# ArjunNarayanan/ProximalPolicyOptimization.jl

Hardware: AMD Instinct MI355X
Metric: env-steps/sec end-to-end PPO (rollout+GAE+update), 4096 envs, 1/2/4/8 MI355X (higher is better)
Workload: dtype f32; 1 GPU; 4096 parallel synthetic rand-poly-shaped envs per GPU (Q=8,H=32,A=128,F=72 int8), 2x256 MLP policy fp32, T=128 steps/iteration, 4 epochs, minibatch 4096/GPU, gamma=1.0 eps=0.05 entropy_w=0.01 Adam 1e-4; returns mode (lambda=1,V=0); envs_per_gpu=4096, T=128, epochs=4, minibatch_per_gpu=4096, parallelism=dp1, rollouts_streamed_to_disk=False

## Files before the change

### proximalpolicyoptimization.jl_amd/csrc/ppo_policy_fwd_x6.hip

```cpp
#include "ppo_policy_tail.h"
#include "ppo_x6.h"
#include <cstdlib>

#define X6F_LANE() unsigned ln = (unsigned)lane; asm volatile("" : "+v"(ln)); const int j = (int)(ln & 31u), h = (int)(ln >> 5); (void)j; (void)h

template <int HID>
struct FXCfg {
    static constexpr int F = 72, NT = HID / 32, KS = HID / 16, K1 = 5;
    static constexpr size_t oFr = 0, szFr = (size_t)NT * 6 * 1024;
    static constexpr size_t oP = oFr + szFr, oW3 = oP + (size_t)NT * 1024, oB1 = oW3 + (size_t)2 * NT * 256,
                            oB2 = oB1 + (size_t)NT * 128, total = oB2 + (size_t)NT * 128;
    static constexpr int WG_PER_CU = HID == 256 ? 2 : 4;
    static_assert(total * WG_PER_CU <= 160 * 1024, "LDS budget");
};

template <int HID>
__global__ __launch_bounds__(HID * 2, 4) void k_policy_fwd_train_x6(FwdArgs a, const uint4* __restrict__ w1x, const uint4* __restrict__ w2fx, int x_by_tile) {
    using C = FXCfg<HID>;
    constexpr int F = C::F, NT = C::NT, KS = C::KS, K1 = C::K1;
    extern __shared__ __attribute__((aligned(16))) char smem_c[];
    char* const frag = smem_c + C::oFr;
    float4* const sP = reinterpret_cast<float4*>(smem_c + C::oP);
    float4* const sW3p = reinterpret_cast<float4*>(smem_c + C::oW3);
    float4* const sB1 = reinterpret_cast<float4*>(smem_c + C::oB1);
    float4* const sB2 = reinterpret_cast<float4*>(smem_c + C::oB2);
    const int tid = threadIdx.x, lane = tid & 63;
    const int w = __builtin_amdgcn_readfirstlane(tid >> 6);
#ifdef PPO_X6_ZERO_LDS
    for (int i = tid; i < (int)(C::total / 4); i += NT * 64) reinterpret_cast<uint32_t*>(smem_c)[i] = 0u;
    __syncthreads();
#endif
    for (int i = tid; i < 2 * NT * 16; i += NT * 64) sW3p[i] = a.w3p[i];
    for (int i = tid; i < NT * 8; i += NT * 64) { sB1[i] = a.b1p[i]; sB2[i] = a.b2p[i]; }
    __syncthreads();
    const char* const w1s = reinterpret_cast<const char*>(w1x + (size_t)w * K1 * 3 * 64);
    const char* const w2s = reinterpret_cast<const char*>(w2fx + (size_t)w * KS * 3 * 64);
    char* const fown = frag + (size_t)w * 6 * 1024;

    uint2 xr[K1];
    auto load_x = [&](int64_t rec, unsigned ln) {
        const char* row = reinterpret_cast<const char*>(a.states) + (size_t)rec * 32 * F + (ln & 31u) * (unsigned)F + (ln >> 5) * 8u;
#pragma unroll
        for (int s = 0; s < K1; ++s) {
            const bool pad = (s == K1 - 1) && (ln >> 5);
            const uint2 v = *reinterpret_cast<const uint2*>(row + (pad ? 0 : 16 * s));
            xr[s] = pad ? make_uint2(0u, 0u) : v;
        }
    };
    int32_t sid = 0;
    if ((int64_t)blockIdx.x < a.B) { sid = __builtin_amdgcn_readfirstlane(a.idx[blockIdx.x]); load_x(x_by_tile ? (int64_t)blockIdx.x : (int64_t)sid, (unsigned)lane); }

    for (int64_t tile = blockIdx.x; tile < a.B; tile += gridDim.x) {
        const uint32_t act = a.active[sid];
        const int32_t sid_cur = sid;
        {
            X6F_LANE();
            unsigned lo16 = ln * 16u;
            constexpr int R1 = 8;
            uint4 ring[R1];
#pragma unroll
            for (int g = 0; g < R1; ++g) ring[g] = *reinterpret_cast<const uint4*>(w1s + (lo16 + (unsigned)g * 1024u));
            f32x16 acc;
#pragma unroll
            for (int q = 0; q < 4; ++q) {
                const float4 b = sB1[(w * 2 + h) * 4 + q];
                acc[4 * q + 0] = b.x; acc[4 * q + 1] = b.y; acc[4 * q + 2] = b.z; acc[4 * q + 3] = b.w;
            }
            uint4 xb[K1];
#pragma unroll
            for (int s = 0; s < K1; ++s) {
                float v[8];
#pragma unroll
                for (int e = 0; e < 8; ++e) v[e] = (float)(int)(int8_t)((e < 4 ? xr[s].x : xr[s].y) >> (8 * (e & 3)));
                xb[s] = make_uint4(x_perm(v[0], v[1]), x_perm(v[2], v[3]), x_perm(v[4], v[5]), x_perm(v[6], v[7]));
            }
            f32x16 accs;
#pragma unroll
            for (int r = 0; r < 16; ++r) accs[r] = 0.0f;
#pragma unroll
            for (int st = 0; st < 3 * K1; ++st) {
                if (st % 3 == 2) acc = x_mfma(ring[st % R1], xb[st / 3], acc);
                else accs = x_mfma(ring[st % R1], xb[st / 3], accs);
                __builtin_amdgcn_sched_barrier(0);
                if (st + R1 < 3 * K1) ring[st % R1] = *reinterpret_cast<const uint4*>(w1s + (lo16 + (unsigned)(st + R1) * 1024u));
                __builtin_amdgcn_sched_barrier(0);
            }
#pragma unroll
            for (int r = 0; r < 16; ++r) acc[r] = acc[r] + accs[r];
            asm volatile("" : "+v"(acc));
            lrelu16(acc);
            float4* dst = a.act1 + ((size_t)tile * NT + w) * 4 * 64;
#pragma unroll
            for (int q = 0; q < 4; ++q) {
                typedef float f32x4l __attribute__((ext_vector_type(4)));
                const f32x4l t = {acc[4 * q], acc[4 * q + 1], acc[4 * q + 2], acc[4 * q + 3]};
                __builtin_nontemporal_store(t, reinterpret_cast<f32x4l*>(dst + q * 64 + ln));
            }
#pragma unroll
            for (int s = 0; s < 2; ++s) {
                uint2 zh[2], zm[2], zl[2];
#pragma unroll
                for (int qq = 0; qq < 2; ++qq) {
                    const int q = 2 * s + qq;
                    const float hv[4] = {acc[4 * q], acc[4 * q + 1], acc[4 * q + 2], acc[4 * q + 3]};
                    x_split4(hv, zh[qq], zm[qq], zl[qq]);
                }
                *reinterpret_cast<uint4*>(fown + (s * 3 + 0) * 1024 + ln * 16) = make_uint4(zh[0].x, zh[0].y, zh[1].x, zh[1].y);
                *reinterpret_cast<uint4*>(fown + (s * 3 + 1) * 1024 + ln * 16) = make_uint4(zm[0].x, zm[0].y, zm[1].x, zm[1].y);
                *reinterpret_cast<uint4*>(fown + (s * 3 + 2) * 1024 + ln * 16) = make_uint4(zl[0].x, zl[0].y, zl[1].x, zl[1].y);
            }
        }
        constexpr int RD = 6;
        static_assert(RD % 3 == 0 && KS % (RD / 3) == 0, "ring rounds");
        static_assert(RD * 1024 <= PPO_X6_W2_PAD_BYTES, "the last ring round reads RD pieces past the end of the W2 stream");
        uint4 ring[RD];
        {
            unsigned lo = (unsigned)lane * 16u;
            asm volatile("" : "+v"(lo));
#pragma unroll
            for (int g = 0; g < RD; ++g) ring[g] = *reinterpret_cast<const uint4*>(w2s + (lo + (unsigned)g * 1024u));
        }
        const int64_t ntile = (tile + gridDim.x < a.B) ? tile + gridDim.x : tile;
        {
            unsigned ln2 = (unsigned)lane;
            asm volatile("" : "+v"(ln2));
            sid = __builtin_amdgcn_readfirstlane(a.idx[ntile]);
            load_x(x_by_tile ? ntile : (int64_t)sid, ln2);
        }
        __syncthreads();
        {
            X6F_LANE();
            f32x16 acc;
#pragma unroll
            for (int q = 0; q < 4; ++q) {
                const float4 b = sB2[(w * 2 + h) * 4 + q];
                acc[4 * q + 0] = b.x; acc[4 * q + 1] = b.y; acc[4 * q + 2] = b.z; acc[4 * q + 3] = b.w;
            }
            f32x16 accm, accl;
#pragma unroll
            for (int r = 0; r < 16; ++r) { accm[r] = 0.0f; accl[r] = 0.0f; }
            const unsigned lo16 = ln * 16u;
            const char* zp = frag + lo16;
            const char* wn = w2s + (size_t)RD * 1024;
#pragma unroll 1
            for (int k0 = 0; k0 < KS; k0 += RD / 3) {
#pragma unroll
                for (int u = 0; u < RD / 3; ++u) {
                    const uint4 z_h = *reinterpret_cast<const uint4*>(zp + (u * 3 + 0) * 1024);
                    const uint4 z_m = *reinterpret_cast<const uint4*>(zp + (u * 3 + 1) * 1024);
                    const uint4 z_l = *reinterpret_cast<const uint4*>(zp + (u * 3 + 2) * 1024);
                    accl = x_mfma(ring[3 * u + 0], z_h, accl);
                    __builtin_amdgcn_sched_barrier(0);
                    ring[3 * u + 0] = *reinterpret_cast<const uint4*>(wn + lo16);
                    __builtin_amdgcn_sched_barrier(0);
                    accl = x_mfma(ring[3 * u + 1], z_m, accl);
                    accm = x_mfma(ring[3 * u + 1], z_h, accm);
                    __builtin_amdgcn_sched_barrier(0);
                    ring[3 * u + 1] = *reinterpret_cast<const uint4*>(wn + 1024 + lo16);
                    __builtin_amdgcn_sched_barrier(0);
                    accl = x_mfma(ring[3 * u + 2], z_l, accl);
                    accm = x_mfma(ring[3 * u + 2], z_m, accm);
                    acc = x_mfma(ring[3 * u + 2], z_h, acc);
                    __builtin_amdgcn_sched_barrier(0);
                    ring[3 * u + 2] = *reinterpret_cast<const uint4*>(wn + 2048 + lo16);
                    wn += 3 * 1024;
                    __builtin_amdgcn_sched_barrier(0);
                }
                zp += (RD / 3) * 3 * 1024;
            }
#pragma unroll
            for (int r = 0; r < 16; ++r) acc[r] = acc[r] + (accm[r] + accl[r]);
            asm volatile("" : "+v"(acc));
            lrelu16(acc);
            float4* dst = a.act2 + ((size_t)tile * NT + w) * 4 * 64;
#pragma unroll
            for (int q = 0; q < 4; ++q) {
                typedef float f32x4l __attribute__((ext_vector_type(4)));
                const f32x4l t = {acc[4 * q], acc[4 * q + 1], acc[4 * q + 2], acc[4 * q + 3]};
                __builtin_nontemporal_store(t, reinterpret_cast<f32x4l*>(dst + q * 64 + ln));
            }
            float p0 = 0.f, p1 = 0.f, p2 = 0.f, p3 = 0.f;
            const float4* w3 = sW3p + (h * NT + w) * 16;
#pragma unroll
            for (int r = 0; r < 16; ++r) {
                const float4 wv = w3[r];
                p0 = fmaf(wv.x, acc[r], p0); p1 = fmaf(wv.y, acc[r], p1);
                p2 = fmaf(wv.z, acc[r], p2); p3 = fmaf(wv.w, acc[r], p3);
            }
            sP[w * 64 + ln] = make_float4(p0, p1, p2, p3);
        }
        __syncthreads();
        if (w == 0) {
            X6F_LANE();
            float4 s = sP[ln];
#pragma unroll
            for (int u = 1; u < NT; ++u) { const float4 q4 = sP[u * 64 + ln]; s.x += q4.x; s.y += q4.y; s.z += q4.z; s.w += q4.w; }
            float l[1][4];
            l[0][0] = (s.x + __shfl_xor(s.x, 32)) + a.b3[0];
            l[0][1] = (s.y + __shfl_xor(s.y, 32)) + a.b3[1];
            l[0][2] = (s.z + __shfl_xor(s.z, 32)) + a.b3[2];
            l[0][3] = (s.w + __shfl_xor(s.w, 32)) + a.b3[3];
            policy_tail<2, 1, false>(a, tile, sid_cur, act, l, (int)ln, j, h);
        }
    }
}

template <int HID, int T>
struct FXTCfg {
    static constexpr int F = 72, NT = HID / 32, KS = HID / 16, K1 = 5;
    static constexpr size_t oFr = 0, szFr = (size_t)T * NT * 6 * 1024;
    static constexpr size_t oP = oFr + szFr, oW3 = oP + (size_t)T * NT * 1024, oB1 = oW3 + (size_t)2 * NT * 256,
                            oB2 = oB1 + (size_t)NT * 128, total = oB2 + (size_t)NT * 128;
    static_assert(total <= 160 * 1024, "LDS budget");
};

template <int HID, int T>
__global__ __launch_bounds__(HID * 2, 2) void k_policy_fwd_train_x6t(FwdArgs a, const uint4* __restrict__ w1x, const uint4* __restrict__ w2fx, int x_by_tile) {
    using C = FXTCfg<HID, T>;
    constexpr int F = C::F, NT = C::NT, KS = C::KS, K1 = C::K1;
    static_assert(T <= NT, "one tail wave per tile");
    static_assert(T == 2, "two scalar id loads per pass; waves 0 and 1 run the tails");
    extern __shared__ __attribute__((aligned(16))) char smem_c[];
    char* const frag = smem_c + C::oFr;
    float4* const sP = reinterpret_cast<float4*>(smem_c + C::oP);
    float4* const sW3p = reinterpret_cast<float4*>(smem_c + C::oW3);
    float4* const sB1 = reinterpret_cast<float4*>(smem_c + C::oB1);
    float4* const sB2 = reinterpret_cast<float4*>(smem_c + C::oB2);
    const int tid = threadIdx.x, lane = tid & 63;
    const int w = __builtin_amdgcn_readfirstlane(tid >> 6);
#ifdef PPO_FX6_STAMP
    unsigned long long st_sum[8] = {0, 0, 0, 0, 0, 0, 0, 0}, st_t = clock64();
#define FXSTAMP(i) do { unsigned long long _n = clock64(); st_sum[i] += _n - st_t; st_t = _n; } while (0)
#else
#define FXSTAMP(i) do { } while (0)
#endif
    const float b3_0 = a.b3[0], b3_1 = a.b3[1], b3_2 = a.b3[2], b3_3 = a.b3[3];
    for (int i = tid; i < 2 * NT * 16; i += NT * 64) sW3p[i] = a.w3p[i];
    for (int i = tid; i < NT * 8; i += NT * 64) { sB1[i] = a.b1p[i]; sB2[i] = a.b2p[i]; }
    __syncthreads();
    const char* const w1s = reinterpret_cast<const char*>(w1x + (size_t)w * K1 * 3 * 64);
    const char* const w2s = reinterpret_cast<const char*>(w2fx + (size_t)w * KS * 3 * 64);

    uint2 xr[T][K1];
    auto load_x = [&](int i, int64_t rec, unsigned ln) {
        const uint64_t rb = x_uniform_addr(reinterpret_cast<const char*>(a.states) + (size_t)rec * 32 * F);
        const unsigned row = (ln & 31u) * (unsigned)F + (ln >> 5) * 8u;
#pragma unroll
        for (int s = 0; s < K1; ++s) {
            const bool pad = (s == K1 - 1) && (ln >> 5);
            unsigned ro = row + (pad ? 0u : 16u * s);
            asm volatile("" : "+v"(ro));
            typedef unsigned u32x2l __attribute__((ext_vector_type(2)));
            const u32x2l vv = *x_gptr<const u32x2l>(rb, ro);
            const uint2 v = make_uint2(vv.x, vv.y);
            xr[i][s] = pad ? make_uint2(0u, 0u) : v;
        }
    };
    auto tile_of = [&](int64_t g, int i) { const int64_t t = g * T + i; return t < a.B ? t : a.B - 1; };
    int cid[T] = {0, 0}, nid[T] = {0, 0};
    auto sload_ids = [&](int64_t g, int (&id)[T]) {
        const int32_t* const ip0 = a.idx + tile_of(g, 0);
        const int32_t* const ip1 = a.idx + tile_of(g, 1);
        asm volatile("s_load_dword %0, %2, 0x0\n\ts_load_dword %1, %3, 0x0\n\ts_waitcnt lgkmcnt(0)"
                     : "=&s"(id[0]), "=&s"(id[1]) : "s"(ip0), "s"(ip1) : "memory");
    };
    uint32_t tact = 0u, nact = 0u;
    TailPre tpre = {0, 0.0f, 0.0f}, npre = {0, 0.0f, 0.0f};
    auto load_tail_in = [&](const int (&id)[T], uint32_t& act, TailPre& pre) {
        const int32_t s = w == 1 ? id[1] : id[0];
        act = a.active[s]; pre.ab = a.actions[s]; pre.po = a.p_old[s]; pre.adv = a.adv[s];
    };
    if ((int64_t)blockIdx.x * T < a.B) {
        sload_ids(blockIdx.x, cid);
#pragma unroll
        for (int i = 0; i < T; ++i) load_x(i, x_by_tile ? tile_of(blockIdx.x, i) : (int64_t)cid[i], (unsigned)lane);
        load_tail_in(cid, tact, tpre);
    }
    for (int64_t g = blockIdx.x; g * T < a.B; g += gridDim.x) {
        {
            X6F_LANE();
            unsigned lo16 = ln * 16u;
            constexpr int R1 = 8;
            uint4 ring[R1];
#pragma unroll
            for (int q = 0; q < R1; ++q) ring[q] = *reinterpret_cast<const uint4*>(w1s + (lo16 + (unsigned)q * 1024u));
            f32x16 acc[T], accs[T];
            uint4 xb[T][K1];
#pragma unroll
            for (int i = 0; i < T; ++i) {
#pragma unroll
                for (int q = 0; q < 4; ++q) {
                    const float4 b = sB1[(w * 2 + h) * 4 + q];
                    acc[i][4 * q + 0] = b.x; acc[i][4 * q + 1] = b.y; acc[i][4 * q + 2] = b.z; acc[i][4 * q + 3] = b.w;
                }
#pragma unroll
                for (int r = 0; r < 16; ++r) accs[i][r] = 0.0f;
#pragma unroll
                for (int s = 0; s < K1; ++s) {
                    float v[8];
#pragma unroll
                    for (int e = 0; e < 8; ++e) v[e] = (float)(int)(int8_t)((e < 4 ? xr[i][s].x : xr[i][s].y) >> (8 * (e & 3)));
                    xb[i][s] = make_uint4(x_perm(v[0], v[1]), x_perm(v[2], v[3]), x_perm(v[4], v[5]), x_perm(v[6], v[7]));
                }
            }
#pragma unroll
            for (int st = 0; st < 3 * K1; ++st) {
#pragma unroll
                for (int i = 0; i < T; ++i) {
                    if (st % 3 == 2) acc[i] = x_mfma(ring[st % R1], xb[i][st / 3], acc[i]);
                    else accs[i] = x_mfma(ring[st % R1], xb[i][st / 3], accs[i]);
                }
                __builtin_amdgcn_sched_barrier(0);
                if (st + R1 < 3 * K1) ring[st % R1] = *reinterpret_cast<const uint4*>(w1s + (lo16 + (unsigned)(st + R1) * 1024u));
                __builtin_amdgcn_sched_barrier(0);
            }
            FXSTAMP(0);
#pragma unroll
            for (int i = 0; i < T; ++i) {
#pragma unroll
                for (int r = 0; r < 16; ++r) acc[i][r] = acc[i][r] + accs[i][r];
                asm volatile("" : "+v"(acc[i]));
                lrelu16(acc[i]);
                const int64_t tile = g * T + i;
                if (tile < a.B) {
                    const uint64_t dst = x_uniform_addr(a.act1 + ((size_t)tile * NT + w) * 4 * 64);
#pragma unroll
                    for (int q = 0; q < 4; ++q) {
                        typedef float f32x4l __attribute__((ext_vector_type(4)));
                        const f32x4l t = {acc[i][4 * q], acc[i][4 * q + 1], acc[i][4 * q + 2], acc[i][4 * q + 3]};
                        unsigned so = ln * 16u + (unsigned)q * 1024u;
                        asm volatile("" : "+v"(so));
                        __builtin_nontemporal_store(t, x_gptr<f32x4l>(dst, so));
                    }
                }
                char* const fown = frag + ((size_t)i * NT + w) * 6 * 1024;
#pragma unroll
                for (int s = 0; s < 2; ++s) {
                    uint2 zh[2], zm[2], zl[2];
#pragma unroll
                    for (int qq = 0; qq < 2; ++qq) {
                        const int q = 2 * s + qq;
                        const float hv[4] = {acc[i][4 * q], acc[i][4 * q + 1], acc[i][4 * q + 2], acc[i][4 * q + 3]};
                        x_split4(hv, zh[qq], zm[qq], zl[qq]);
                    }
                    *reinterpret_cast<uint4*>(fown + (s * 3 + 0) * 1024 + ln * 16) = make_uint4(zh[0].x, zh[0].y, zh[1].x, zh[1].y);
                    *reinterpret_cast<uint4*>(fown + (s * 3 + 1) * 1024 + ln * 16) = make_uint4(zm[0].x, zm[0].y, zm[1].x, zm[1].y);
                    *reinterpret_cast<uint4*>(fown + (s * 3 + 2) * 1024 + ln * 16) = make_uint4(zl[0].x, zl[0].y, zl[1].x, zl[1].y);
                }
            }
        }
        FXSTAMP(1);
        constexpr int RD = 6;
        static_assert(KS % (RD / 3) == 0, "ring rounds");
        static_assert(RD * 1024 <= PPO_X6_W2_PAD_BYTES, "the last ring round reads RD pieces past the end of the W2 stream");
        uint4 ring[RD];
        {
            unsigned lo = (unsigned)lane * 16u;
            asm volatile("" : "+v"(lo));
#pragma unroll
            for (int q = 0; q < RD; ++q) ring[q] = *reinterpret_cast<const uint4*>(w2s + (lo + (unsigned)q * 1024u));
        }
        {
            const int64_t gn = ((g + gridDim.x) * T < a.B) ? g + gridDim.x : g;
            unsigned ln2 = (unsigned)lane;
            asm volatile("" : "+v"(ln2));
            sload_ids(gn, nid);
#pragma unroll
            for (int i = 0; i < T; ++i) load_x(i, x_by_tile ? tile_of(gn, i) : (int64_t)nid[i], ln2);
            load_tail_in(nid, nact, npre);
        }
        FXSTAMP(2);
        __syncthreads();
        FXSTAMP(3);
        {
            X6F_LANE();
            f32x16 acc[T], accs[T];
#pragma unroll
            for (int i = 0; i < T; ++i) {
#pragma unroll
                for (int q = 0; q < 4; ++q) {
                    const float4 b = sB2[(w * 2 + h) * 4 + q];
                    acc[i][4 * q + 0] = b.x; acc[i][4 * q + 1] = b.y; acc[i][4 * q + 2] = b.z; acc[i][4 * q + 3] = b.w;
                }
#pragma unroll
                for (int r = 0; r < 16; ++r) accs[i][r] = 0.0f;
            }
            const unsigned lo16 = ln * 16u;
            const char* zp = frag + lo16;
            unsigned wo = (unsigned)RD * 1024u;
            asm volatile("" : "+s"(wo));
#pragma unroll 1
            for (int k0 = 0; k0 < KS; k0 += RD / 3) {
#pragma unroll
                for (int u = 0; u < RD / 3; ++u) {
                    const uint4 wl = ring[3 * u + 0], wm = ring[3 * u + 1], wh = ring[3 * u + 2];
#pragma unroll
                    for (int i = 0; i < T; ++i) {
                        const char* zi = zp + (size_t)i * NT * 6 * 1024;
                        const uint4 z_h = *reinterpret_cast<const uint4*>(zi + (u * 3 + 0) * 1024);
                        const uint4 z_m = *reinterpret_cast<const uint4*>(zi + (u * 3 + 1) * 1024);
                        const uint4 z_l = *reinterpret_cast<const uint4*>(zi + (u * 3 + 2) * 1024);
                        accs[i] = x_mfma(wl, z_h, accs[i]);
                        accs[i] = x_mfma(wm, z_m, accs[i]);
                        accs[i] = x_mfma(wm, z_h, accs[i]);
                        accs[i] = x_mfma(wh, z_l, accs[i]);
                        accs[i] = x_mfma(wh, z_m, accs[i]);
                        acc[i] = x_mfma(wh, z_h, acc[i]);
                    }
                    __builtin_amdgcn_sched_barrier(0);
                    ring[3 * u + 0] = *reinterpret_cast<const uint4*>(w2s + (lo16 + wo));
                    ring[3 * u + 1] = *reinterpret_cast<const uint4*>(w2s + (lo16 + wo + 1024u));
                    ring[3 * u + 2] = *reinterpret_cast<const uint4*>(w2s + (lo16 + wo + 2048u));
                    wo += 3 * 1024;
                    asm volatile("" : "+s"(wo));
                    __builtin_amdgcn_sched_barrier(0);
                }
                zp += (RD / 3) * 3 * 1024;
            }
            FXSTAMP(4);
#pragma unroll
            for (int i = 0; i < T; ++i) {
#pragma unroll
                for (int r = 0; r < 16; ++r) acc[i][r] = acc[i][r] + accs[i][r];
                asm volatile("" : "+v"(acc[i]));
                lrelu16(acc[i]);
                const int64_t tile = g * T + i;
                if (tile < a.B) {
                    const uint64_t dst = x_uniform_addr(a.act2 + ((size_t)tile * NT + w) * 4 * 64);
#pragma unroll
                    for (int q = 0; q < 4; ++q) {
                        typedef float f32x4l __attribute__((ext_vector_type(4)));
                        const f32x4l t = {acc[i][4 * q], acc[i][4 * q + 1], acc[i][4 * q + 2], acc[i][4 * q + 3]};
                        unsigned so = ln * 16u + (unsigned)q * 1024u;
                        asm volatile("" : "+v"(so));
                        __builtin_nontemporal_store(t, x_gptr<f32x4l>(dst, so));
                    }
                }
                float p0 = 0.f, p1 = 0.f, p2 = 0.f, p3 = 0.f;
                const float4* w3 = sW3p + (h * NT + w) * 16;
#pragma unroll
                for (int r = 0; r < 16; ++r) {
                    const float4 wv = w3[r];
                    p0 = fmaf(wv.x, acc[i][r], p0); p1 = fmaf(wv.y, acc[i][r], p1);
                    p2 = fmaf(wv.z, acc[i][r], p2); p3 = fmaf(wv.w, acc[i][r], p3);
                }
                sP[(i * NT + w) * 64 + ln] = make_float4(p0, p1, p2, p3);
            }
        }
        FXSTAMP(5);
        __syncthreads();
        FXSTAMP(6);
        if (w < T && g * T + w < a.B) {
            X6F_LANE();
            const int64_t tile = g * T + w;
            const int32_t sidw = w == 0 ? cid[0] : cid[1];
            const float4* sPi = sP + (size_t)w * NT * 64;
            float4 s = sPi[ln];
#pragma unroll
            for (int u = 1; u < NT; ++u) { const float4 q4 = sPi[u * 64 + ln]; s.x += q4.x; s.y += q4.y; s.z += q4.z; s.w += q4.w; }
            float l[1][4];
            l[0][0] = (s.x + __shfl_xor(s.x, 32)) + b3_0;
            l[0][1] = (s.y + __shfl_xor(s.y, 32)) + b3_1;
            l[0][2] = (s.z + __shfl_xor(s.z, 32)) + b3_2;
            l[0][3] = (s.w + __shfl_xor(s.w, 32)) + b3_3;
            policy_tail<2, 1, false>(a, tile, sidw, tact, l, (int)ln, j, h, 0u, 0, &tpre);
        }
        FXSTAMP(7);
        cid[0] = nid[0]; cid[1] = nid[1];
        tact = nact; tpre = npre;
    }
#ifdef PPO_FX6_STAMP
    if (a.stamps && lane == 0 && (w == 0 || w == NT - 1))
        for (int i = 0; i < 8; ++i) a.stamps[((size_t)blockIdx.x * 2 + (w ? 1 : 0)) * 8 + i] = st_sum[i];
#endif
#undef FXSTAMP
}

template <int HID, int TPS>
struct FXSCfg {
    static constexpr int F = 72, NT = HID / 32, KS = HID / 16, K1 = 5;
    static constexpr size_t oFr = 0, szFr = (size_t)2 * NT * 6 * 1024;
    static constexpr size_t oP = oFr + szFr, oW3 = oP + (size_t)TPS * NT * 1024, oB1 = oW3 + (size_t)2 * NT * 256,
                            oB2 = oB1 + (size_t)NT * 128, total = oB2 + (size_t)NT * 128;
    static_assert(total <= 160 * 1024, "LDS budget");
};

template <int HID, int TPS>
__global__ __launch_bounds__(HID * 2, 2) void k_policy_fwd_train_x6s(FwdArgs a, const uint4* __restrict__ w1x, const uint4* __restrict__ w2fx, int x_by_tile) {
    constexpr int T = 2;
    static_assert(TPS % T == 0, "tiles of a state in pairs");
    using C = FXSCfg<HID, TPS>;
    constexpr int F = C::F, NT = C::NT, KS = C::KS, K1 = C::K1;
    extern __shared__ __attribute__((aligned(16))) char smem_c[];
    char* const frag = smem_c + C::oFr;
    float4* const sP = reinterpret_cast<float4*>(smem_c + C::oP);
    float4* const sW3p = reinterpret_cast<float4*>(smem_c + C::oW3);
    float4* const sB1 = reinterpret_cast<float4*>(smem_c + C::oB1);
    float4* const sB2 = reinterpret_cast<float4*>(smem_c + C::oB2);
    const int tid = threadIdx.x, lane = tid & 63;
    const int w = __builtin_amdgcn_readfirstlane(tid >> 6);
    for (int i = tid; i < 2 * NT * 16; i += NT * 64) sW3p[i] = a.w3p[i];
    for (int i = tid; i < NT * 8; i += NT * 64) { sB1[i] = a.b1p[i]; sB2[i] = a.b2p[i]; }
    __syncthreads();
    const char* const w1s = reinterpret_cast<const char*>(w1x + (size_t)w * K1 * 3 * 64);
    const char* const w2s = reinterpret_cast<const char*>(w2fx + (size_t)w * KS * 3 * 64);

    uint2 xr[T][K1];
    auto load_x = [&](int i, int64_t rec, unsigned ln) {
        const char* row = reinterpret_cast<const char*>(a.states) + (size_t)rec * 32 * F + (ln & 31u) * (unsigned)F + (ln >> 5) * 8u;
#pragma unroll
        for (int s = 0; s < K1; ++s) {
            const bool pad = (s == K1 - 1) && (ln >> 5);
            const uint2 v = *reinterpret_cast<const uint2*>(row + (pad ? 0 : 16 * s));
            xr[i][s] = pad ? make_uint2(0u, 0u) : v;
        }
    };
    constexpr int NP = TPS / T;
    auto rec_of = [&](int64_t state, int ts) {
        return (x_by_tile ? state : (int64_t)__builtin_amdgcn_readfirstlane(a.idx[state])) * TPS + ts;
    };
    if ((int64_t)blockIdx.x < a.B) {
#pragma unroll
        for (int i = 0; i < T; ++i) load_x(i, rec_of(blockIdx.x, i), (unsigned)lane);
    }
    for (int64_t st8 = blockIdx.x; st8 < a.B; st8 += gridDim.x) {
    for (int p = 0; p < NP; ++p) {
        const int64_t g = st8 * NP + p;
        {
            X6F_LANE();
            unsigned lo16 = ln * 16u;
            constexpr int R1 = 8;
            uint4 ring[R1];
#pragma unroll
            for (int q = 0; q < R1; ++q) ring[q] = *reinterpret_cast<const uint4*>(w1s + (lo16 + (unsigned)q * 1024u));
            f32x16 acc[T], accs[T];
            uint4 xb[T][K1];
#pragma unroll
            for (int i = 0; i < T; ++i) {
#pragma unroll
                for (int q = 0; q < 4; ++q) {
                    const float4 b = sB1[(w * 2 + h) * 4 + q];
                    acc[i][4 * q + 0] = b.x; acc[i][4 * q + 1] = b.y; acc[i][4 * q + 2] = b.z; acc[i][4 * q + 3] = b.w;
                }
#pragma unroll
                for (int r = 0; r < 16; ++r) accs[i][r] = 0.0f;
#pragma unroll
                for (int s = 0; s < K1; ++s) {
                    float v[8];
#pragma unroll
                    for (int e = 0; e < 8; ++e) v[e] = (float)(int)(int8_t)((e < 4 ? xr[i][s].x : xr[i][s].y) >> (8 * (e & 3)));
                    xb[i][s] = make_uint4(x_perm(v[0], v[1]), x_perm(v[2], v[3]), x_perm(v[4], v[5]), x_perm(v[6], v[7]));
                }
            }
#pragma unroll
            for (int st = 0; st < 3 * K1; ++st) {
#pragma unroll
                for (int i = 0; i < T; ++i) {
                    if (st % 3 == 2) acc[i] = x_mfma(ring[st % R1], xb[i][st / 3], acc[i]);
                    else accs[i] = x_mfma(ring[st % R1], xb[i][st / 3], accs[i]);
                }
                __builtin_amdgcn_sched_barrier(0);
                if (st + R1 < 3 * K1) ring[st % R1] = *reinterpret_cast<const uint4*>(w1s + (lo16 + (unsigned)(st + R1) * 1024u));
                __builtin_amdgcn_sched_barrier(0);
            }
#pragma unroll
            for (int i = 0; i < T; ++i) {
#pragma unroll
                for (int r = 0; r < 16; ++r) acc[i][r] = acc[i][r] + accs[i][r];
                asm volatile("" : "+v"(acc[i]));
                lrelu16(acc[i]);
                const int64_t tile = g * T + i;
                {
                    float4* dst = a.act1 + ((size_t)tile * NT + w) * 4 * 64;
#pragma unroll
                    for (int q = 0; q < 4; ++q) {
                        typedef float f32x4l __attribute__((ext_vector_type(4)));
                        const f32x4l t = {acc[i][4 * q], acc[i][4 * q + 1], acc[i][4 * q + 2], acc[i][4 * q + 3]};
                        __builtin_nontemporal_store(t, reinterpret_cast<f32x4l*>(dst + q * 64 + ln));
                    }
                }
                char* const fown = frag + ((size_t)i * NT + w) * 6 * 1024;
#pragma unroll
                for (int s = 0; s < 2; ++s) {
                    uint2 zh[2], zm[2], zl[2];
#pragma unroll
                    for (int qq = 0; qq < 2; ++qq) {
                        const int q = 2 * s + qq;
                        const float hv[4] = {acc[i][4 * q], acc[i][4 * q + 1], acc[i][4 * q + 2], acc[i][4 * q + 3]};
                        x_split4(hv, zh[qq], zm[qq], zl[qq]);
                    }
                    *reinterpret_cast<uint4*>(fown + (s * 3 + 0) * 1024 + ln * 16) = make_uint4(zh[0].x, zh[0].y, zh[1].x, zh[1].y);
                    *reinterpret_cast<uint4*>(fown + (s * 3 + 1) * 1024 + ln * 16) = make_uint4(zm[0].x, zm[0].y, zm[1].x, zm[1].y);
                    *reinterpret_cast<uint4*>(fown + (s * 3 + 2) * 1024 + ln * 16) = make_uint4(zl[0].x, zl[0].y, zl[1].x, zl[1].y);
                }
            }
        }
        constexpr int RD = 6;
        static_assert(KS % (RD / 3) == 0, "ring rounds");
        uint4 ring[RD];
        {
            unsigned lo = (unsigned)lane * 16u;
            asm volatile("" : "+v"(lo));
#pragma unroll
            for (int q = 0; q < RD; ++q) ring[q] = *reinterpret_cast<const uint4*>(w2s + (lo + (unsigned)q * 1024u));
        }
        {
            const bool more = p + 1 < NP;
            const int64_t sn = more ? st8 : (st8 + gridDim.x < a.B ? st8 + gridDim.x : st8);
            const int pn = more ? p + 1 : (st8 + gridDim.x < a.B ? 0 : p);
            unsigned ln2 = (unsigned)lane;
            asm volatile("" : "+v"(ln2));
#pragma unroll
            for (int i = 0; i < T; ++i) load_x(i, rec_of(sn, pn * T + i), ln2);
        }
        __syncthreads();
        {
            X6F_LANE();
            f32x16 acc[T], accs[T];
#pragma unroll
            for (int i = 0; i < T; ++i) {
#pragma unroll
                for (int q = 0; q < 4; ++q) {
                    const float4 b = sB2[(w * 2 + h) * 4 + q];
                    acc[i][4 * q + 0] = b.x; acc[i][4 * q + 1] = b.y; acc[i][4 * q + 2] = b.z; acc[i][4 * q + 3] = b.w;
                }
#pragma unroll
                for (int r = 0; r < 16; ++r) accs[i][r] = 0.0f;
            }
            const unsigned lo16 = ln * 16u;
            const char* zp = frag + lo16;
            const char* wn = w2s + (size_t)RD * 1024;
#pragma unroll 1
            for (int k0 = 0; k0 < KS; k0 += RD / 3) {
#pragma unroll
                for (int u = 0; u < RD / 3; ++u) {
                    const uint4 wl = ring[3 * u + 0], wm = ring[3 * u + 1], wh = ring[3 * u + 2];
#pragma unroll
                    for (int i = 0; i < T; ++i) {
                        const char* zi = zp + (size_t)i * NT * 6 * 1024;
                        const uint4 z_h = *reinterpret_cast<const uint4*>(zi + (u * 3 + 0) * 1024);
                        const uint4 z_m = *reinterpret_cast<const uint4*>(zi + (u * 3 + 1) * 1024);
                        const uint4 z_l = *reinterpret_cast<const uint4*>(zi + (u * 3 + 2) * 1024);
                        accs[i] = x_mfma(wl, z_h, accs[i]);
                        accs[i] = x_mfma(wm, z_m, accs[i]);
                        accs[i] = x_mfma(wm, z_h, accs[i]);
                        accs[i] = x_mfma(wh, z_l, accs[i]);
                        accs[i] = x_mfma(wh, z_m, accs[i]);
                        acc[i] = x_mfma(wh, z_h, acc[i]);
                    }
                    __builtin_amdgcn_sched_barrier(0);
                    ring[3 * u + 0] = *reinterpret_cast<const uint4*>(wn + lo16);
                    ring[3 * u + 1] = *reinterpret_cast<const uint4*>(wn + 1024 + lo16);
                    ring[3 * u + 2] = *reinterpret_cast<const uint4*>(wn + 2048 + lo16);
                    wn += 3 * 1024;
                    __builtin_amdgcn_sched_barrier(0);
                }
                zp += (RD / 3) * 3 * 1024;
            }
#pragma unroll
            for (int i = 0; i < T; ++i) {
#pragma unroll
                for (int r = 0; r < 16; ++r) acc[i][r] = acc[i][r] + accs[i][r];
                asm volatile("" : "+v"(acc[i]));
                lrelu16(acc[i]);
                const int64_t tile = g * T + i;
                {
                    float4* dst = a.act2 + ((size_t)tile * NT + w) * 4 * 64;
#pragma unroll
                    for (int q = 0; q < 4; ++q) {
                        typedef float f32x4l __attribute__((ext_vector_type(4)));
                        const f32x4l t = {acc[i][4 * q], acc[i][4 * q + 1], acc[i][4 * q + 2], acc[i][4 * q + 3]};
                        __builtin_nontemporal_store(t, reinterpret_cast<f32x4l*>(dst + q * 64 + ln));
                    }
                }
                float p0 = 0.f, p1 = 0.f, p2 = 0.f, p3 = 0.f;
                const float4* w3 = sW3p + (h * NT + w) * 16;
#pragma unroll
                for (int r = 0; r < 16; ++r) {
                    const float4 wv = w3[r];
                    p0 = fmaf(wv.x, acc[i][r], p0); p1 = fmaf(wv.y, acc[i][r], p1);
                    p2 = fmaf(wv.z, acc[i][r], p2); p3 = fmaf(wv.w, acc[i][r], p3);
                }
                sP[((p * T + i) * NT + w) * 64 + ln] = make_float4(p0, p1, p2, p3);
            }
        }
        __syncthreads();
        if (p == NP - 1 && w == 0) {
            X6F_LANE();
            const int32_t sidw = __builtin_amdgcn_readfirstlane(a.idx[st8]);
            const uint32_t act = a.active[sidw];
            float l[TPS][4];
#pragma unroll
            for (int ts = 0; ts < TPS; ++ts) {
                const float4* sPi = sP + (size_t)ts * NT * 64;
                float4 s = sPi[ln];
#pragma unroll
                for (int u = 1; u < NT; ++u) { const float4 q4 = sPi[u * 64 + ln]; s.x += q4.x; s.y += q4.y; s.z += q4.z; s.w += q4.w; }
                l[ts][0] = (s.x + __shfl_xor(s.x, 32)) + a.b3[0];
                l[ts][1] = (s.y + __shfl_xor(s.y, 32)) + a.b3[1];
                l[ts][2] = (s.z + __shfl_xor(s.z, 32)) + a.b3[2];
                l[ts][3] = (s.w + __shfl_xor(s.w, 32)) + a.b3[3];
            }
            policy_tail<2, TPS, false>(a, st8, sidw, act, l, (int)ln, j, h);
        }
    }
    }
}

#ifdef PPO_FX6_STAMP
static unsigned long long* g_fx6_stamps = nullptr;
extern "C" int32_t ppo_debug_fx6_stamps(unsigned long long* out) {
    if (!g_fx6_stamps) return -1;
    (void)hipDeviceSynchronize();
    return hipMemcpy(out, g_fx6_stamps, 512 * 2 * 8 * 8, hipMemcpyDeviceToHost) == hipSuccess ? 0 : -2;
}
#endif

int32_t launch_policy_train_fwd_x6(ppo_policy_s* p, FwdArgs& a, int64_t B, TrainFwd form, bool compact) {
#ifdef PPO_FX6_STAMP
    if (!g_fx6_stamps) { (void)hipMalloc((void**)&g_fx6_stamps, 512 * 2 * 8 * 8); (void)hipMemset(g_fx6_stamps, 0, 512 * 2 * 8 * 8); }
    a.stamps = g_fx6_stamps;
#endif
    if (compact) {
        PPO_TRY(launch_expand_states(a.cstate, a.active, a.env_tmpl, B, a.envQ, a.xs_out, a.idx));
        a.states = a.xs_out;
    }
#define LAUNCH(K, LDS, GROUPS, CAP, THREADS)                                                                 \
    do {                                                                                                     \
        const int64_t groups = GROUPS, cap = CAP;                                                            \
        const int nwg = (int)(groups < cap ? groups : cap);                                                  \
        static thread_local bool attr_set = false;                                                           \
        if (!attr_set) {                                                                                     \
            HIP_TRY(hipFuncSetAttribute((const void*)K, hipFuncAttributeMaxDynamicSharedMemorySize, (int)LDS)); \
            attr_set = true;                                                                                 \
        }                                                                                                    \
        hipLaunchKernelGGL(K, dim3(nwg), dim3(THREADS), LDS, ppo_stream(), a,                                \
                           (const uint4*)p->w1x.p, (const uint4*)p->w2fx.p, compact ? 1 : 0);                 \
    } while (0)
    if (form == TrainFwd::X6S) LAUNCH((k_policy_fwd_train_x6s<256, 4>), (FXSCfg<256, 4>::total), B, 256, 512);
    else if (form == TrainFwd::X6T && p->HID == 256) LAUNCH((k_policy_fwd_train_x6t<256, 2>), (FXTCfg<256, 2>::total), (B + 1) / 2, 256, 512);
    else if (form == TrainFwd::X6T) LAUNCH((k_policy_fwd_train_x6t<128, 2>), (FXTCfg<128, 2>::total), (B + 1) / 2, 512, 256);
    else if (p->HID == 256) LAUNCH(k_policy_fwd_train_x6<256>, FXCfg<256>::total, B, 256 * FXCfg<256>::WG_PER_CU, 512);
    else LAUNCH(k_policy_fwd_train_x6<128>, FXCfg<128>::total, B, 256 * FXCfg<128>::WG_PER_CU, 256);
#undef LAUNCH
    HIP_TRY(hipGetLastError());
    return PPO_OK;
}
```

Measured before the change: 2.439 million env-steps/s.

## Add helper waves to x6t forward for X prefetch/convert and policy tail

For HID=256 the x6t training-forward kernel gains two extra helper waves per workgroup. Each helper prefetches the next tile's int8 state rows, converts them to the MFMA operand layout in LDS, and runs the policy tail for one tile, so the compute waves no longer do input loads, int8 conversion or tail work. This adds an extra LDS X image, extra barriers between helpers and compute waves, and changes the launch-bounds occupancy hint from 2 to 1 workgroup per CU. Whether it runs depends on the X6T form being selected.

```diff
diff --git a/proximalpolicyoptimization.jl_amd/csrc/ppo_policy_fwd_x6.hip b/proximalpolicyoptimization.jl_amd/csrc/ppo_policy_fwd_x6.hip
--- a/proximalpolicyoptimization.jl_amd/csrc/ppo_policy_fwd_x6.hip
+++ b/proximalpolicyoptimization.jl_amd/csrc/ppo_policy_fwd_x6.hip
@@ -208,26 +208,35 @@
 template <int HID, int T>
 struct FXTCfg {
     static constexpr int F = 72, NT = HID / 32, KS = HID / 16, K1 = 5;
+    static constexpr bool HELP = HID == 256;
+    static constexpr int WAVES = NT + (HELP ? T : 0), THREADS = WAVES * 64;
     static constexpr size_t oFr = 0, szFr = (size_t)T * NT * 6 * 1024;
     static constexpr size_t oP = oFr + szFr, oW3 = oP + (size_t)T * NT * 1024, oB1 = oW3 + (size_t)2 * NT * 256,
-                            oB2 = oB1 + (size_t)NT * 128, total = oB2 + (size_t)NT * 128;
-    static_assert(total <= 160 * 1024, "LDS budget");
+                            oB2 = oB1 + (size_t)NT * 128, oX = oB2 + (size_t)NT * 128,
+                            total = oX + (HELP ? (size_t)T * K1 * 1024 : 0);
+    static constexpr int WG_PER_CU = HID == 256 ? 1 : 2;
+    static_assert(total * WG_PER_CU <= 160 * 1024, "LDS budget");
+    static_assert(oX % 16 == 0, "ds_read_b128 / ds_write_b128 alignment of the X image");
 };
 
 template <int HID, int T>
-__global__ __launch_bounds__(HID * 2, 2) void k_policy_fwd_train_x6t(FwdArgs a, const uint4* __restrict__ w1x, const uint4* __restrict__ w2fx, int x_by_tile) {
+__global__ __launch_bounds__((FXTCfg<HID, T>::THREADS), (FXTCfg<HID, T>::WG_PER_CU)) void k_policy_fwd_train_x6t(FwdArgs a, const uint4* __restrict__ w1x, const uint4* __restrict__ w2fx, int x_by_tile) {
     using C = FXTCfg<HID, T>;
     constexpr int F = C::F, NT = C::NT, KS = C::KS, K1 = C::K1;
+    constexpr bool HELP = C::HELP;
     static_assert(T <= NT, "one tail wave per tile");
-    static_assert(T == 2, "two scalar id loads per pass; waves 0 and 1 run the tails");
+    static_assert(T == 2, "two scalar id loads per pass; two waves run the tails");
     extern __shared__ __attribute__((aligned(16))) char smem_c[];
     char* const frag = smem_c + C::oFr;
     float4* const sP = reinterpret_cast<float4*>(smem_c + C::oP);
     float4* const sW3p = reinterpret_cast<float4*>(smem_c + C::oW3);
     float4* const sB1 = reinterpret_cast<float4*>(smem_c + C::oB1);
     float4* const sB2 = reinterpret_cast<float4*>(smem_c + C::oB2);
+    uint4* const sX = reinterpret_cast<uint4*>(smem_c + C::oX);
     const int tid = threadIdx.x, lane = tid & 63;
     const int w = __builtin_amdgcn_readfirstlane(tid >> 6);
+    const bool helper = HELP && w >= NT;
+    const int hi = helper ? w - NT : 0;
 #ifdef PPO_FX6_STAMP
     unsigned long long st_sum[8] = {0, 0, 0, 0, 0, 0, 0, 0}, st_t = clock64();
 #define FXSTAMP(i) do { unsigned long long _n = clock64(); st_sum[i] += _n - st_t; st_t = _n; } while (0)
@@ -235,14 +244,13 @@
 #define FXSTAMP(i) do { } while (0)
 #endif
     const float b3_0 = a.b3[0], b3_1 = a.b3[1], b3_2 = a.b3[2], b3_3 = a.b3[3];
-    for (int i = tid; i < 2 * NT * 16; i += NT * 64) sW3p[i] = a.w3p[i];
-    for (int i = tid; i < NT * 8; i += NT * 64) { sB1[i] = a.b1p[i]; sB2[i] = a.b2p[i]; }
-    __syncthreads();
+    for (int i = tid; i < 2 * NT * 16; i += C::THREADS) sW3p[i] = a.w3p[i];
+    for (int i = tid; i < NT * 8; i += C::THREADS) { sB1[i] = a.b1p[i]; sB2[i] = a.b2p[i]; }
     const char* const w1s = reinterpret_cast<const char*>(w1x + (size_t)w * K1 * 3 * 64);
     const char* const w2s = reinterpret_cast<const char*>(w2fx + (size_t)w * KS * 3 * 64);
 
-    uint2 xr[T][K1];
-    auto load_x = [&](int i, int64_t rec, unsigned ln) {
+    uint2 xr[K1];
+    auto load_x = [&](int64_t rec, unsigned ln) {
         const uint64_t rb = x_uniform_addr(reinterpret_cast<const char*>(a.states) + (size_t)rec * 32 * F);
         const unsigned row = (ln & 31u) * (unsigned)F + (ln >> 5) * 8u;
 #pragma unroll
@@ -253,28 +261,105 @@
             typedef unsigned u32x2l __attribute__((ext_vector_type(2)));
             const u32x2l vv = *x_gptr<const u32x2l>(rb, ro);
             const uint2 v = make_uint2(vv.x, vv.y);
-            xr[i][s] = pad ? make_uint2(0u, 0u) : v;
+            xr[s] = pad ? make_uint2(0u, 0u) : v;
+        }
+    };
+    auto write_x = [&](unsigned ln) {
+        uint4* const dst = sX + (size_t)hi * K1 * 64;
+#pragma unroll
+        for (int s = 0; s < K1; ++s) {
+            float v[8];
+#pragma unroll
+            for (int e = 0; e < 8; ++e) v[e] = (float)(int)(int8_t)((e < 4 ? xr[s].x : xr[s].y) >> (8 * (e & 3)));
+            dst[s * 64 + ln] = make_uint4(x_perm(v[0], v[1]), x_perm(v[2], v[3]), x_perm(v[4], v[5]), x_perm(v[6], v[7]));
         }
     };
     auto tile_of = [&](int64_t g, int i) { const int64_t t = g * T + i; return t < a.B ? t : a.B - 1; };
-    int cid[T] = {0, 0}, nid[T] = {0, 0};
-    auto sload_ids = [&](int64_t g, int (&id)[T]) {
+    int cid = 0, nid = 0;
+    auto sload_id = [&](int64_t g, int& id) {
+        const int32_t* const ip = a.idx + tile_of(g, hi);
+        asm volatile("s_load_dword %0, %1, 0x0\n\ts_waitcnt lgkmcnt(0)" : "=&s"(id) : "s"(ip) : "memory");
+    };
+    uint32_t tact = 0u, nact = 0u;
+    TailPre tpre = {0, 0.0f, 0.0f}, npre = {0, 0.0f, 0.0f};
+    auto load_tail_in = [&](const int id, uint32_t& act, TailPre& pre) {
+        act = a.active[id]; pre.ab = a.actions[id]; pre.po = a.p_old[id]; pre.adv = a.adv[id];
+    };
+    uint2 cxr[T][K1];
+    auto c_load_x = [&](int i, int64_t rec, unsigned ln) {
+        const uint64_t rb = x_uniform_addr(reinterpret_cast<const char*>(a.states) + (size_t)rec * 32 * F);
+        const unsigned row = (ln & 31u) * (unsigned)F + (ln >> 5) * 8u;
+#pragma unroll
+        for (int s = 0; s < K1; ++s) {
+            const bool pad = (s == K1 - 1) && (ln >> 5);
+            unsigned ro = row + (pad ? 0u : 16u * s);
+            asm volatile("" : "+v"(ro));
+            typedef unsigned u32x2l __attribute__((ext_vector_type(2)));
+            const u32x2l vv = *x_gptr<const u32x2l>(rb, ro);
+            const uint2 v = make_uint2(vv.x, vv.y);
+            cxr[i][s] = pad ? make_uint2(0u, 0u) : v;
+        }
+    };
+    int ccid[T] = {0, 0}, cnid[T] = {0, 0};
+    auto c_sload_ids = [&](int64_t g, int (&id)[T]) {
         const int32_t* const ip0 = a.idx + tile_of(g, 0);
         const int32_t* const ip1 = a.idx + tile_of(g, 1);
         asm volatile("s_load_dword %0, %2, 0x0\n\ts_load_dword %1, %3, 0x0\n\ts_waitcnt lgkmcnt(0)"
                      : "=&s"(id[0]), "=&s"(id[1]) : "s"(ip0), "s"(ip1) : "memory");
     };
-    uint32_t tact = 0u, nact = 0u;
-    TailPre tpre = {0, 0.0f, 0.0f}, npre = {0, 0.0f, 0.0f};
-    auto load_tail_in = [&](const int (&id)[T], uint32_t& act, TailPre& pre) {
-        const int32_t s = w == 1 ? id[1] : id[0];
-        act = a.active[s]; pre.ab = a.actions[s]; pre.po = a.p_old[s]; pre.adv = a.adv[s];
-    };
-    if ((int64_t)blockIdx.x * T < a.B) {
-        sload_ids(blockIdx.x, cid);
-#pragma unroll
-        for (int i = 0; i < T; ++i) load_x(i, x_by_tile ? tile_of(blockIdx.x, i) : (int64_t)cid[i], (unsigned)lane);
+    auto c_load_tail_in = [&](const int (&id)[T], uint32_t& act, TailPre& pre) { load_tail_in(w == 1 ? id[1] : id[0], act, pre); };
+    if (!HELP && (int64_t)blockIdx.x * T < a.B) {
+        c_sload_ids(blockIdx.x, ccid);
+#pragma unroll
+        for (int i = 0; i < T; ++i) c_load_x(i, x_by_tile ? tile_of(blockIdx.x, i) : (int64_t)ccid[i], (unsigned)lane);
+        c_load_tail_in(ccid, tact, tpre);
+    }
+    if (helper && (int64_t)blockIdx.x * T < a.B) {
+        sload_id(blockIdx.x, cid);
+        load_x(x_by_tile ? tile_of(blockIdx.x, hi) : (int64_t)cid, (unsigned)lane);
         load_tail_in(cid, tact, tpre);
+        write_x((unsigned)lane);
+    }
+    __syncthreads();
+#ifdef PPO_FX6_STAMP
+#define FXSTORE() do { if (a.stamps && lane == 0 && (w == 0 || w == NT - 1 || w == NT))      \
+        for (int i = 0; i < 8; ++i) a.stamps[((size_t)blockIdx.x * 3 + (w == 0 ? 0 : w == NT - 1 ? 1 : 2)) * 8 + i] = st_sum[i]; } while (0)
+#else
+#define FXSTORE() do { } while (0)
+#endif
+    if (helper) {
+        for (int64_t g = blockIdx.x; g * T < a.B; g += gridDim.x) {
+            __syncthreads();
+            FXSTAMP(0);
+            const int64_t gn = ((g + gridDim.x) * T < a.B) ? g + gridDim.x : g;
+            X6F_LANE();
+            sload_id(gn, nid);
+            load_x(x_by_tile ? tile_of(gn, hi) : (int64_t)nid, ln);
+            load_tail_in(nid, nact, npre);
+            FXSTAMP(1);
+            write_x(ln);
+            FXSTAMP(2);
+            __syncthreads();
+            FXSTAMP(3);
+            if (g * T + hi < a.B) {
+                const int64_t tile = g * T + hi;
+                const float4* sPi = sP + (size_t)hi * NT * 64;
+                float4 s = sPi[ln];
+#pragma unroll
+                for (int u = 1; u < NT; ++u) { const float4 q4 = sPi[u * 64 + ln]; s.x += q4.x; s.y += q4.y; s.z += q4.z; s.w += q4.w; }
+                float l[1][4];
+                l[0][0] = (s.x + __shfl_xor(s.x, 32)) + b3_0;
+                l[0][1] = (s.y + __shfl_xor(s.y, 32)) + b3_1;
+                l[0][2] = (s.z + __shfl_xor(s.z, 32)) + b3_2;
+                l[0][3] = (s.w + __shfl_xor(s.w, 32)) + b3_3;
+                policy_tail<2, 1, false>(a, tile, cid, tact, l, (int)ln, j, h, 0u, 0, &tpre);
+            }
+            FXSTAMP(4);
+            cid = nid;
+            tact = nact; tpre = npre;
+        }
+        FXSTORE();
+        return;
     }
     for (int64_t g = blockIdx.x; g * T < a.B; g += gridDim.x) {
         {
@@ -297,9 +382,10 @@
                 for (int r = 0; r < 16; ++r) accs[i][r] = 0.0f;
 #pragma unroll
                 for (int s = 0; s < K1; ++s) {
+                    if (HELP) { xb[i][s] = sX[(i * K1 + s) * 64 + ln]; continue; }
                     float v[8];
 #pragma unroll
-                    for (int e = 0; e < 8; ++e) v[e] = (float)(int)(int8_t)((e < 4 ? xr[i][s].x : xr[i][s].y) >> (8 * (e & 3)));
+                    for (int e = 0; e < 8; ++e) v[e] = (float)(int)(int8_t)((e < 4 ? cxr[i][s].x : cxr[i][s].y) >> (8 * (e & 3)));
                     xb[i][s] = make_uint4(x_perm(v[0], v[1]), x_perm(v[2], v[3]), x_perm(v[4], v[5]), x_perm(v[6], v[7]));
                 }
             }
@@ -360,14 +446,14 @@
 #pragma unroll
             for (int q = 0; q < RD; ++q) ring[q] = *reinterpret_cast<const uint4*>(w2s + (lo + (unsigned)q * 1024u));
         }
-        {
+        if (!HELP) {
             const int64_t gn = ((g + gridDim.x) * T < a.B) ? g + gridDim.x : g;
             unsigned ln2 = (unsigned)lane;
             asm volatile("" : "+v"(ln2));
-            sload_ids(gn, nid);
-#pragma unroll
-            for (int i = 0; i < T; ++i) load_x(i, x_by_tile ? tile_of(gn, i) : (int64_t)nid[i], ln2);
-            load_tail_in(nid, nact, npre);
+            c_sload_ids(gn, cnid);
+#pragma unroll
+            for (int i = 0; i < T; ++i) c_load_x(i, x_by_tile ? tile_of(gn, i) : (int64_t)cnid[i], ln2);
+            c_load_tail_in(cnid, nact, npre);
         }
         FXSTAMP(2);
         __syncthreads();
@@ -450,29 +536,29 @@
         FXSTAMP(5);
         __syncthreads();
         FXSTAMP(6);
-        if (w < T && g * T + w < a.B) {
-            X6F_LANE();
-            const int64_t tile = g * T + w;
-            const int32_t sidw = w == 0 ? cid[0] : cid[1];
-            const float4* sPi = sP + (size_t)w * NT * 64;
-            float4 s = sPi[ln];
-#pragma unroll
-            for (int u = 1; u < NT; ++u) { const float4 q4 = sPi[u * 64 + ln]; s.x += q4.x; s.y += q4.y; s.z += q4.z; s.w += q4.w; }
-            float l[1][4];
-            l[0][0] = (s.x + __shfl_xor(s.x, 32)) + b3_0;
-            l[0][1] = (s.y + __shfl_xor(s.y, 32)) + b3_1;
-            l[0][2] = (s.z + __shfl_xor(s.z, 32)) + b3_2;
-            l[0][3] = (s.w + __shfl_xor(s.w, 32)) + b3_3;
-            policy_tail<2, 1, false>(a, tile, sidw, tact, l, (int)ln, j, h, 0u, 0, &tpre);
-        }
-        FXSTAMP(7);
-        cid[0] = nid[0]; cid[1] = nid[1];
-        tact = nact; tpre = npre;
+        if (!HELP) {
+            if (w < T && g * T + w < a.B) {
+                X6F_LANE();
+                const int64_t tile = g * T + w;
+                const int32_t sidw = w == 0 ? ccid[0] : ccid[1];
+                const float4* sPi = sP + (size_t)w * NT * 64;
+                float4 s = sPi[ln];
+#pragma unroll
+                for (int u = 1; u < NT; ++u) { const float4 q4 = sPi[u * 64 + ln]; s.x += q4.x; s.y += q4.y; s.z += q4.z; s.w += q4.w; }
+                float l[1][4];
+                l[0][0] = (s.x + __shfl_xor(s.x, 32)) + b3_0;
+                l[0][1] = (s.y + __shfl_xor(s.y, 32)) + b3_1;
+                l[0][2] = (s.z + __shfl_xor(s.z, 32)) + b3_2;
+                l[0][3] = (s.w + __shfl_xor(s.w, 32)) + b3_3;
+                policy_tail<2, 1, false>(a, tile, sidw, tact, l, (int)ln, j, h, 0u, 0, &tpre);
+            }
+            FXSTAMP(7);
+            ccid[0] = cnid[0]; ccid[1] = cnid[1];
+            tact = nact; tpre = npre;
+        }
     }
-#ifdef PPO_FX6_STAMP
-    if (a.stamps && lane == 0 && (w == 0 || w == NT - 1))
-        for (int i = 0; i < 8; ++i) a.stamps[((size_t)blockIdx.x * 2 + (w ? 1 : 0)) * 8 + i] = st_sum[i];
-#endif
+    FXSTORE();
+#undef FXSTORE
 #undef FXSTAMP
 }
 
@@ -712,13 +798,13 @@
 extern "C" int32_t ppo_debug_fx6_stamps(unsigned long long* out) {
     if (!g_fx6_stamps) return -1;
     (void)hipDeviceSynchronize();
-    return hipMemcpy(out, g_fx6_stamps, 512 * 2 * 8 * 8, hipMemcpyDeviceToHost) == hipSuccess ? 0 : -2;
+    return hipMemcpy(out, g_fx6_stamps, 512 * 3 * 8 * 8, hipMemcpyDeviceToHost) == hipSuccess ? 0 : -2;
 }
 #endif
 
 int32_t launch_policy_train_fwd_x6(ppo_policy_s* p, FwdArgs& a, int64_t B, TrainFwd form, bool compact) {
 #ifdef PPO_FX6_STAMP
-    if (!g_fx6_stamps) { (void)hipMalloc((void**)&g_fx6_stamps, 512 * 2 * 8 * 8); (void)hipMemset(g_fx6_stamps, 0, 512 * 2 * 8 * 8); }
+    if (!g_fx6_stamps) { (void)hipMalloc((void**)&g_fx6_stamps, 512 * 3 * 8 * 8); (void)hipMemset(g_fx6_stamps, 0, 512 * 3 * 8 * 8); }
     a.stamps = g_fx6_stamps;
 #endif
     if (compact) {
@@ -738,8 +824,8 @@
                            (const uint4*)p->w1x.p, (const uint4*)p->w2fx.p, compact ? 1 : 0);                 \
     } while (0)
     if (form == TrainFwd::X6S) LAUNCH((k_policy_fwd_train_x6s<256, 4>), (FXSCfg<256, 4>::total), B, 256, 512);
-    else if (form == TrainFwd::X6T && p->HID == 256) LAUNCH((k_policy_fwd_train_x6t<256, 2>), (FXTCfg<256, 2>::total), (B + 1) / 2, 256, 512);
-    else if (form == TrainFwd::X6T) LAUNCH((k_policy_fwd_train_x6t<128, 2>), (FXTCfg<128, 2>::total), (B + 1) / 2, 512, 256);
+    else if (form == TrainFwd::X6T && p->HID == 256) LAUNCH((k_policy_fwd_train_x6t<256, 2>), (FXTCfg<256, 2>::total), (B + 1) / 2, 256, (FXTCfg<256, 2>::THREADS));
+    else if (form == TrainFwd::X6T) LAUNCH((k_policy_fwd_train_x6t<128, 2>), (FXTCfg<128, 2>::total), (B + 1) / 2, 512, (FXTCfg<128, 2>::THREADS));
     else if (p->HID == 256) LAUNCH(k_policy_fwd_train_x6<256>, FXCfg<256>::total, B, 256 * FXCfg<256>::WG_PER_CU, 512);
     else LAUNCH(k_policy_fwd_train_x6<128>, FXCfg<128>::total, B, 256 * FXCfg<128>::WG_PER_CU, 256);
 #undef LAUNCH
```

Measured after the change: 2.468 million env-steps/s (median of 6 runs). 1.01x the previous value.
